# MengLcool/RichSem

Hardware: AMD Instinct MI355X
Metric: training images/sec, RichSem R50 4-scale 1333x800 (MSDeformAttn hot path: 12 fwd + 12 bwd calls per step) (higher is better)
Workload: dtype f32; 1 GPU; configs[1]: R50 4-scale 800x1344 (S=22323), bs=2/GPU, M=8 D=32 L=P=4; per step 6x E(Lq=22323) + 6x Dd(Lq=1092), forward and backward, 12 distinct per-layer tensor sets; loc-init; loc=init, images_per_gpu=2, parallelism=dp1 (replicas, no collective)

## Files before the change

richsem_amd/csrc/msda_rps.h:

```cpp
#pragma once

#include <algorithm>
#include <atomic>
#include <vector>

#include "msda_common.h"

namespace msda {

constexpr int kRpsThreads = 768;
constexpr int kRpsWaves = kRpsThreads / 64;
constexpr int kRpsMaxPx = 256;
constexpr int kRpsPpq = (kRpsMaxPx + kRpsThreads / 4 - 1) / (kRpsThreads / 4);
constexpr int kRpsRpl = 2;
constexpr int kRpsChunk = kRpsRpl * kRpsThreads;
constexpr int kRpsSumStride = 36;
constexpr int kRpsSegShift = 3;
constexpr int kRpsMaxSegs = kRpsMaxPx + (kRpsChunk >> kRpsSegShift);
constexpr int kRpsMaxL = 4;
constexpr int kRpsMaxUnits = 448;
constexpr int kRpsD = 32;
constexpr int kRpsPad = 32;
constexpr int kRpsDummyWgs = 2048, kRpsDummyBytes = kRpsDummyWgs * 1024;
constexpr int kRpsMaxRuns = 320;
constexpr int kRpsRunSearch = 256;
static_assert(kRpsRunSearch < kRpsMaxRuns && 2 * kRpsRunSearch >= kRpsMaxRuns, "run search");
constexpr int kRpsQpBits = 19;
static_assert(kRpsMaxPx <= 256, "record code: the base-grid index has 8 bits (bits 19..26), the tile kernel masks it with 0xFF");

struct RpsLevel {
    int H, W, start;
    int TH, TW, nty, ntx;
    int bin0;
    int nslab;
    int atomic;
    float inv_TH, inv_TW;
};

struct alignas(16) RpsRec {
    unsigned code;
    float lh, lw, a;
};

struct RpsGeom {
    int N, S, M, Lq, L, P;
    int nunits, ppx;
    int bins_per_pair, nbins;
    RpsLevel lv[kRpsMaxL];
    unsigned units[kRpsMaxUnits];
    unsigned *ctr;
    unsigned long long *bin_state;
    uint2 *runs;
    int max_runs;
    int route_threads;
    unsigned entries_cap;
    struct RpsRec *entries;
    int lut_r[kRpsMaxL], lut_c[kRpsMaxL], lut_n;
    int seg_shift;
    float *dummy;
    unsigned long long *stamps;
};

struct alignas(16) RpsEnt {
    float lh;
    float hwa, lwa;
    unsigned row;
};

struct RpsLds {
    int item_slot[2];
    int wave_tot[16];
    int n_segs, pad[3];
    int uhist[16];
    uint2 runs[kRpsMaxRuns];
    unsigned long long stamp_last, stamp_acc[14];
    int offs[kRpsMaxPx + 4];
    unsigned short seg[kRpsMaxSegs + 16];
    RpsEnt ent[kRpsChunk];
    RpsRec meta[kRpsChunk];
    unsigned short slot[kRpsChunk];
    double sum[kRpsMaxPx * kRpsSumStride];
    float vtile[kRpsMaxPx * kRpsD];
};
static_assert(sizeof(RpsLds) <= 160 * 1024, "rps: LDS budget");

__device__ __forceinline__ int rps_wave_scan(int v)
{
    v += __builtin_amdgcn_update_dpp(0, v, 0x111, 0xF, 0xF, true);
    v += __builtin_amdgcn_update_dpp(0, v, 0x112, 0xF, 0xF, true);
    v += __builtin_amdgcn_update_dpp(0, v, 0x114, 0xF, 0xF, true);
    v += __builtin_amdgcn_update_dpp(0, v, 0x118, 0xF, 0xF, true);
    v += __builtin_amdgcn_update_dpp(0, v, 0x142, 0xA, 0xF, false);
    v += __builtin_amdgcn_update_dpp(0, v, 0x143, 0xC, 0xF, false);
    return v;
}

#define RPS_STAMP(i)                                                                   \
    if (kStamps && g.stamps && threadIdx.x == 0) {                                     \
        const unsigned long long now_ = __builtin_amdgcn_s_memtime();                  \
        S->stamp_acc[i] += now_ - S->stamp_last;                                       \
        S->stamp_last = now_;                                                          \
    }

__device__ __forceinline__ unsigned rps_lut_row(const RpsLevel &v, int r)
{
    const int h_low = r - 1, br = max(h_low, 0);
    const int ty = (int)(((float)br + 0.5f) * v.inv_TH);
    const int R0 = ty * v.TH;
    const unsigned gr = (unsigned)(h_low - R0 + 1);
    const unsigned inr = (h_low >= 0 ? 1u : 0u) | (h_low + 1 < v.H ? 2u : 0u);
    return gr | inr << 6 | (unsigned)(ty * v.ntx * v.nslab) << 8;
}
__device__ __forceinline__ unsigned rps_lut_col(const RpsLevel &v, int c)
{
    const int w_low = c - 1, bc = max(w_low, 0);
    const int tx = (int)(((float)bc + 0.5f) * v.inv_TW);
    const int C0 = tx * v.TW, C1 = min(v.W, C0 + v.TW);
    const unsigned gc = (unsigned)(w_low - C0 + 1);
    const unsigned inc = (w_low >= 0 ? 1u : 0u) | (w_low + 1 < v.W ? 2u : 0u);
    const unsigned gw = (unsigned)(C1 - C0 + 1);
    return gc | inc << 6 | (unsigned)(tx * v.nslab) << 8 | gw << 17;
}

constexpr int kRpsRouteThreadsMax = 1024;
static_assert(kRpsMaxUnits <= 512, "route pass: one thread per bin of a pair");

template <int kRpsRouteThreads, int kL = 0, int kP = 0, bool kStamps = false>
__global__ __launch_bounds__(kRpsRouteThreads, 4) void rps_route_kernel(const float *__restrict__ loc, const float *__restrict__ aw,
                                                                     float *__restrict__ grad_value, float *__restrict__ grad_loc,
                                                                     float *__restrict__ grad_aw, const RpsGeom g)
{
    __shared__ unsigned hist[kRpsMaxUnits], base[512];
    __shared__ unsigned wtot[kRpsRouteThreads / kWave];
    __shared__ unsigned sink[kWave];
    extern __shared__ unsigned rps_lut[];
    const int tid = threadIdx.x, lane = tid & (kWave - 1), wave = tid / kWave;
    const int B = g.bins_per_pair;
    const int L = kL ? kL : g.L;
    {
        const int gtid = blockIdx.x * blockDim.x + tid, gsz = gridDim.x * blockDim.x;
        if (gtid < 8) g.ctr[gtid] = 0u;
        if (tid < kWave) sink[tid] = 0u;
        const int row4 = g.M * kRpsD / 4;
        for (int l = 0; l < L; ++l) {
            const RpsLevel &v = g.lv[l];
            for (int i = tid; i <= v.H; i += kRpsRouteThreads) rps_lut[g.lut_r[l] + i] = rps_lut_row(v, i);
            for (int i = tid; i <= v.W; i += kRpsRouteThreads) rps_lut[g.lut_c[l] + i] = rps_lut_col(v, i);
            if (!v.atomic) {
                const int nb = v.nty * v.W + v.ntx * v.H;
                for (int b = 0; b < g.N; ++b) {
                    float4 *dst = reinterpret_cast<float4 *>(grad_value) + (size_t)(b * g.S + v.start) * row4;
                    for (int i = gtid; i < nb * row4; i += gsz) {
                        const int k = i / row4, c = i - k * row4;
                        int px;
                        if (k < v.nty * v.W) {
                            const int ty = k / v.W;
                            px = ty * v.TH * v.W + (k - ty * v.W);
                        } else {
                            const int k2 = k - v.nty * v.W, tx = k2 / v.H;
                            px = (k2 - tx * v.H) * v.W + tx * v.TW;
                        }
                        dst[(size_t)px * row4 + c] = make_float4(0.f, 0.f, 0.f, 0.f);
                    }
                }
                continue;
            }
            const int n4 = v.H * v.W * row4;
            for (int b = 0; b < g.N; ++b) {
                float4 *dst = reinterpret_cast<float4 *>(grad_value) + (size_t)(b * g.S + v.start) * row4;
                for (int i = gtid; i < n4; i += gsz) dst[i] = make_float4(0.f, 0.f, 0.f, 0.f);
            }
        }
    }
    const int P = kP ? kP : g.P, LP = L * P;
    const int qpw = P <= 4 ? 16 : (P <= 8 ? 8 : (P <= 16 ? 4 : (P <= 32 ? 2 : 1)));
    const int ql = lane / P, pp = lane - ql * P;
    const int qpb = qpw * (kRpsRouteThreads / kWave);
    const int qblocks = (g.Lq + qpb - 1) / qpb;
    const int pairs = g.N * g.M;
    const int n_items = pairs * qblocks;
    const unsigned long long lt_mask = (1ull << lane) - 1ull;
    unsigned long long st_acc[8] = {0, 0, 0, 0, 0, 0, 0, 0}, st_last = kStamps && g.stamps ? __builtin_amdgcn_s_memtime() : 0ull;
#define RPS_RSTAMP(i)                                                  \
    if (kStamps && g.stamps) {                                         \
        const unsigned long long now_ = __builtin_amdgcn_s_memtime();  \
        st_acc[i] += now_ - st_last;                                   \
        st_last = now_;                                                \
    }
    float2 xy[kRpsMaxL];
    const int step_pair = (int)(gridDim.x % (unsigned)pairs), step_qb = (int)(gridDim.x / (unsigned)pairs);
    auto item_point = [&](int item_, int pair_, int qb_, bool &live_, int &q_) {
        const int b_ = pair_ / g.M, m_ = pair_ - b_ * g.M;
        q_ = qb_ * qpb + wave * qpw + ql;
        live_ = item_ < n_items && ql < qpw && pp < P && q_ < g.Lq;
        return (unsigned)(((b_ * g.Lq + (live_ ? q_ : 0)) * g.M + m_) * LP + min(pp, P - 1));
    };
    auto request_xy = [&](int item_, int pair_, int qb_) {
        bool live_;
        int q_;
        const unsigned pt0_ = item_point(item_, pair_, qb_, live_, q_);
#pragma unroll
        for (int l = 0; l < kRpsMaxL; ++l) xy[l] = *reinterpret_cast<const float2 *>(loc + 2u * (pt0_ + (unsigned)(min(l, L - 1) * P)));
    };
    int pair = (int)(blockIdx.x % (unsigned)pairs), qb = (int)(blockIdx.x / (unsigned)pairs);
    request_xy(blockIdx.x, pair, qb);
    unsigned long long p_old = 0ull;
    unsigned p_first = 0u, p_cnt = 0u;
    size_t p_gb = 0;
    for (int item = blockIdx.x; item < n_items; item += gridDim.x) {
        for (int i = tid; i < B; i += kRpsRouteThreads) hist[i] = 0u;
        bool live;
        int q;
        const unsigned pt0 = item_point(item, pair, qb, live, q);
        int n_pair = pair + step_pair, n_qb = qb + step_qb;
        if (n_pair >= pairs) {
            n_pair -= pairs;
            ++n_qb;
        }
        n_qb = min(n_qb, qblocks - 1);
        __syncthreads();
        RPS_RSTAMP(1)
        unsigned word[kRpsMaxL];
        unsigned inmap[kRpsMaxL];
        float lh[kRpsMaxL], lw[kRpsMaxL];
        unsigned re[kRpsMaxL], ce[kRpsMaxL];
        unsigned valid_m = 0u, asked_m = 0u, matched_m = 0u;
        unsigned dropped = 0u;
#pragma unroll
        for (int l = 0; l < kRpsMaxL; ++l) {
            lh[l] = lw[l] = 0.f;
            re[l] = ce[l] = 0u;
            if (l >= L) continue;
            const RpsLevel &v = g.lv[l];
            const float Hf = (float)v.H, Wf = (float)v.W;
            const float h_im = xy[l].y * Hf - 0.5f, w_im = xy[l].x * Wf - 0.5f;
            const bool valid = live && h_im > -1.f && w_im > -1.f && h_im < Hf && w_im < Wf;
            valid_m |= valid ? 1u << l : 0u;
            const float hf = floorf(h_im), wf = floorf(w_im);
            lh[l] = h_im - hf;
            lw[l] = w_im - wf;
            dropped |= live && !valid ? 1u << l : 0u;
            re[l] = rps_lut[g.lut_r[l] + (valid ? (int)hf + 1 : 0)];
            ce[l] = rps_lut[g.lut_c[l] + (valid ? (int)wf + 1 : 0)];
        }
        request_xy(item + (int)gridDim.x, n_pair, n_qb);
        float at[kRpsMaxL];
#pragma unroll
        for (int l = 0; l < kRpsMaxL; ++l) at[l] = aw[pt0 + (unsigned)(min(l, L - 1) * P)];
        int ob[kRpsMaxL], lead[kRpsMaxL], lb[kRpsMaxL];
        unsigned own_rank[kRpsMaxL], lt_cnt[kRpsMaxL], n_match[kRpsMaxL];
#pragma unroll
        for (int l = 0; l < kRpsMaxL; ++l) {
            ob[l] = -1;
            lead[l] = 0;
            lb[l] = -1;
            own_rank[l] = lt_cnt[l] = n_match[l] = 0u;
            inmap[l] = 0u;
            word[l] = ~0u;
            if (l >= L) continue;
            const RpsLevel &v = g.lv[l];
            const int ns = v.nslab;
            const int slab = ns > 1 ? uni(qb % ns) : 0;
            ob[l] = (valid_m >> l & 1u) ? v.bin0 + slab + (int)(re[l] >> 8) + (int)((ce[l] >> 8) & 511u) : -1;
            const unsigned inr = (re[l] >> 6) & 3u, inc = (ce[l] >> 6) & 3u;
            inmap[l] = ((inr & 1u) ? inc : 0u) | ((inr & 2u) ? inc << 2 : 0u);
            const unsigned long long vote = __ballot(ob[l] >= 0);
            const int ld = vote ? __ffsll((long long)vote) - 1 : 0;
            lb[l] = __builtin_amdgcn_readlane(ob[l], ld);
            const unsigned long long match = __ballot(ob[l] == lb[l]);
            lead[l] = ld;
            matched_m |= ob[l] == lb[l] && lb[l] >= 0 ? 1u << l : 0u;
            lt_cnt[l] = (unsigned)__popcll(match & lt_mask);
            n_match[l] = (unsigned)__popcll(match);
        }
#pragma unroll
        for (int l = 0; l < kRpsMaxL; ++l) {
            const bool is_lead = lane == lead[l] && lb[l] >= 0, other = ob[l] >= 0 && ob[l] != lb[l];
            const bool asked = is_lead || other;
            asked_m |= asked ? 1u << l : 0u;
            own_rank[l] = atomicAdd(asked ? &hist[is_lead ? lb[l] : ob[l]] : &sink[lane], is_lead ? n_match[l] : (other ? 1u : 0u));
        }
#pragma unroll
        for (int l = 0; l < kRpsMaxL; ++l) {
            if (l >= L) continue;
            const unsigned gr = re[l] & 31u, gc = ce[l] & 31u;
            if (!(asked_m >> l & 1u)) own_rank[l] = lt_cnt[l];
            if (ob[l] >= 0) word[l] = (unsigned)ob[l] | (gr * ((ce[l] >> 17) & 31u) + gc) << 23;
        }
        RPS_RSTAMP(2)
        __syncthreads();
        RPS_RSTAMP(3)
        const unsigned cnt = tid < B ? hist[tid] : 0u;
        const unsigned incl = (unsigned)rps_wave_scan((int)cnt);
        if (lane == kWave - 1) wtot[wave] = incl;
        __syncthreads();
        unsigned before = 0u;
#pragma unroll
        for (int w = 0; w < kRpsRouteThreads / kWave; ++w) before += w < wave ? wtot[w] : 0u;
        const unsigned first = (unsigned)item * (unsigned)(qpb * LP) + before + incl - cnt;
        if (cnt) base[tid] = first;
#pragma unroll
        for (int l = 0; l < kRpsMaxL; ++l) {
            if (l >= L) continue;
            unsigned r = own_rank[l];
            const unsigned rl = (unsigned)__builtin_amdgcn_readlane((int)r, lead[l]);
            if ((matched_m >> l & 1u) && lane != lead[l]) r += rl;
            if (word[l] != ~0u) word[l] |= r << 9;
        }
        __syncthreads();
        RPS_RSTAMP(4)
        const size_t gb = (size_t)pair * B + min(tid, B - 1);
        unsigned long long *const scratch64 = reinterpret_cast<unsigned long long *>(g.dummy + (size_t)(blockIdx.x & (kRpsDummyWgs - 1)) * 256) + lane;
        if (p_cnt) g.runs[p_gb * (size_t)g.max_runs + (size_t)min((unsigned)(p_old >> 32), (unsigned)g.max_runs - 1u)] = make_uint2(p_first, (unsigned)p_old);
        const unsigned long long old = atomicAdd(cnt ? g.bin_state + gb * (kRpsPad / 2) : scratch64, cnt ? (1ull << 32) | (unsigned long long)cnt : 0ull);
        const unsigned qp = (unsigned)((live ? q : 0) * P + pp);
        unsigned slot0[kRpsMaxL];
#pragma unroll
        for (int l = 0; l < kRpsMaxL; ++l) slot0[l] = base[word[l] & 511u];
        asm volatile("" : "+v"(at[0]), "+v"(at[1]), "+v"(at[2]), "+v"(at[3]));
#pragma unroll
        for (int l = 0; l < kRpsMaxL; ++l) {
            const unsigned w = word[l];
            if (w != ~0u) {
                const unsigned slot = min(slot0[l] + ((w >> 9) & 16383u), g.entries_cap - 1u);
                const unsigned code = qp | (w >> 23) << kRpsQpBits | inmap[l] << 27 | 0x80000000u;
                g.entries[slot] = RpsRec{code, lh[l], lw[l], at[l]};
            }
        }
        if (__ballot(dropped != 0u)) {
#pragma unroll
            for (int l = 0; l < kRpsMaxL; ++l)
                if (dropped >> l & 1u) {
                    const unsigned pt = pt0 + (unsigned)(l * P);
                    grad_aw[pt] = 0.f;
                    *reinterpret_cast<float2 *>(grad_loc + 2u * pt) = make_float2(0.f, 0.f);
                }
        }
        RPS_RSTAMP(5)
        p_old = old;
        p_first = first;
        p_cnt = cnt;
        p_gb = gb;
        pair = n_pair;
        qb = n_qb;
        RPS_RSTAMP(6)
        __syncthreads();
        RPS_RSTAMP(7)
    }
    if (p_cnt) g.runs[p_gb * (size_t)g.max_runs + (size_t)min((unsigned)(p_old >> 32), (unsigned)g.max_runs - 1u)] = make_uint2(p_first, (unsigned)p_old);
    if (kStamps && g.stamps && tid == 0)
        for (int i = 0; i < 8; ++i) g.stamps[(size_t)(1024 + blockIdx.x) * 16 + i] = st_acc[i];
#undef RPS_RSTAMP
}

typedef float rps_v2f __attribute__((ext_vector_type(2)));
typedef float rps_v4f __attribute__((ext_vector_type(4)));

__device__ __forceinline__ float rps_quad_rotated_sum(float x0, float x1, float x2, float x3)
{
    const float ra = x0 + dpp_f<kDppXor1>(x1);
    const float rb = x2 + dpp_f<kDppXor1>(x3);
    return ra + dpp_f<kDppXor2>(rb);
}

template <typename TV>
struct RpsRow;
template <>
struct RpsRow<float> {
    float4 a, b;
    __device__ __forceinline__ void load(const float *base, unsigned off)
    {
        a = *reinterpret_cast<const float4 *>(reinterpret_cast<const char *>(base) + off);
        b = *reinterpret_cast<const float4 *>(reinterpret_cast<const char *>(base) + off + 64u);
    }
    __device__ __forceinline__ void unpack(rps_v2f (&gq)[4]) const
    {
        gq[0] = (rps_v2f){a.x, a.y}; gq[1] = (rps_v2f){a.z, a.w};
        gq[2] = (rps_v2f){b.x, b.y}; gq[3] = (rps_v2f){b.z, b.w};
    }
};
template <>
struct RpsRow<bf16_t> {
    uint2 a, b;
    __device__ __forceinline__ void load(const bf16_t *base, unsigned off)
    {
        a = *reinterpret_cast<const uint2 *>(reinterpret_cast<const char *>(base) + off);
        b = *reinterpret_cast<const uint2 *>(reinterpret_cast<const char *>(base) + off + 32u);
    }
    __device__ __forceinline__ void unpack(rps_v2f (&gq)[4]) const
    {
        gq[0] = (rps_v2f){__uint_as_float(a.x << 16), __uint_as_float(a.x & 0xFFFF0000u)};
        gq[1] = (rps_v2f){__uint_as_float(a.y << 16), __uint_as_float(a.y & 0xFFFF0000u)};
        gq[2] = (rps_v2f){__uint_as_float(b.x << 16), __uint_as_float(b.x & 0xFFFF0000u)};
        gq[3] = (rps_v2f){__uint_as_float(b.y << 16), __uint_as_float(b.y & 0xFFFF0000u)};
    }
};

template <bool P4, typename TV = float, bool kStamps = false>
__global__ __launch_bounds__(kRpsThreads, kRpsThreads / 256) void rps_tile_kernel(
    const TV *__restrict__ value, const TV *__restrict__ grad_out, TV *__restrict__ grad_value, float *__restrict__ grad_acc,
    float *__restrict__ grad_loc, float *__restrict__ grad_aw, const RpsGeom g)
{
    extern __shared__ __attribute__((aligned(16))) unsigned char smem[];
    RpsLds *S = reinterpret_cast<RpsLds *>(smem);

    const int tid = threadIdx.x, lane = tid & (kWave - 1), wave = tid / kWave;
    const int j4 = tid & 3, quad = tid >> 2;
    const int c_lo = 4 * j4, c_hi = 16 + 4 * j4;
    const float w_ys = (j4 & 2) ? 1.f : -1.f, w_yc = (j4 & 2) ? 0.f : 1.f;
    const unsigned w_xoff = (j4 & 1) ? 8u : 4u;
    const unsigned lane_row = (unsigned)(c_lo * sizeof(TV));
    const int P = P4 ? 4 : g.P;
    const int LP = g.L * P;
    const int row_elems = g.M * kRpsD;
    const int pairs = g.N * g.M;
    const int xq = blockIdx.x & (kXcds - 1);
    const int n_items = g.nunits * g.ppx;
    float *const dummy_w = g.dummy + (size_t)(blockIdx.x & (kRpsDummyWgs - 1)) * 256;
    if (kStamps && g.stamps && tid == 0) {
        for (int i = 0; i < 14; ++i) S->stamp_acc[i] = 0;
        S->stamp_last = __builtin_amdgcn_s_memtime();
    }
    struct Item {
        bool live;
        int l, b, m, H, W, R0, R1, C0, C1, gw, npx;
    };
    auto item_geom = [&](int id) {
        Item it;
        const unsigned unit = (unsigned)uni((int)g.units[min(id, n_items - 1) / g.ppx]);
        const int pr = xq + kXcds * (min(id, n_items - 1) % g.ppx);
        const int pair = min(pr, pairs - 1);
        it.live = id < n_items && pr < pairs;
        it.l = unit & 3;
        const int ty = (unit >> 2) & 63, tx = (unit >> 8) & 63;
        it.b = pair / g.M;
        it.m = pair - it.b * g.M;
        it.H = g.lv[it.l].H;
        it.W = g.lv[it.l].W;
        it.R0 = ty * g.lv[it.l].TH;
        it.R1 = min(it.H, it.R0 + g.lv[it.l].TH);
        it.C0 = tx * g.lv[it.l].TW;
        it.C1 = min(it.W, it.C0 + g.lv[it.l].TW);
        it.gw = it.C1 - it.C0 + 1;
        it.npx = it.live ? (it.R1 - it.R0 + 1) * it.gw : 0;
        return it;
    };
    auto bin_range_raw = [&](int id, unsigned &bin_, unsigned &okm_, unsigned long long &st_) {
        const int idc = min(id, n_items - 1);
        const unsigned unit = g.units[idc / g.ppx];
        const int pair = xq + kXcds * (idc % g.ppx);
        const bool ok = id < n_items && pair < pairs;
        const int l = unit & 3, ty = (unit >> 2) & 63, tx = (unit >> 8) & 63, slab = (unit >> 14) & 255, nslab = (unit >> 22) & 255;
        const unsigned bin_c = ok ? (unsigned)(pair * g.bins_per_pair + g.lv[l].bin0 + (ty * g.lv[l].ntx + tx) * nslab + slab) : 0u;
        st_ = g.bin_state[(size_t)bin_c * (kRpsPad / 2)];
        okm_ = ok ? 0xFFFFFFFFu : 0u;
        bin_ = bin_c | ~okm_;
    };
    auto bin_counts = [&](unsigned long long st_, unsigned okm_, int &n, int &nr) {
        unsigned lo = (unsigned)st_, hi = (unsigned)(st_ >> 32);
        asm volatile("" : "+v"(lo), "+v"(hi));
        n = (int)(min(lo, 0x7FFFFFFFu) & okm_);
        nr = (int)(min(hi, (unsigned)min(g.max_runs, kRpsMaxRuns)) & okm_);
    };
    auto bin_range = [&](int id, unsigned &bin_, int &n, int &nr) {
        const int idc = min(id, n_items - 1);
        const unsigned unit = g.units[idc / g.ppx];
        const int pair = xq + kXcds * (idc % g.ppx);
        const bool ok = id < n_items && pair < pairs;
        const int l = unit & 3, ty = (unit >> 2) & 63, tx = (unit >> 8) & 63, slab = (unit >> 14) & 255, nslab = (unit >> 22) & 255;
        const unsigned bin_c = ok ? (unsigned)(pair * g.bins_per_pair + g.lv[l].bin0 + (ty * g.lv[l].ntx + tx) * nslab + slab) : 0u;
        const unsigned long long st = g.bin_state[(size_t)bin_c * (kRpsPad / 2)];
        const unsigned okm = ok ? 0xFFFFFFFFu : 0u;
        bin_ = bin_c | ~okm;
        n = (int)(min((unsigned)st, 0x7FFFFFFFu) & okm);
        nr = (int)(min((unsigned)(st >> 32), (unsigned)min(g.max_runs, kRpsMaxRuns)) & okm);
    };
    uint2 run_reg = make_uint2(0u, 0u);
    auto load_runs = [&](unsigned bin_, int nr) {
        const int i = min(tid, max(uni(nr) - 1, 0));
        const unsigned b_ = (unsigned)uni((int)bin_);
        run_reg = g.runs[(size_t)(b_ == 0xFFFFFFFFu ? 0u : b_) * g.max_runs + i];
    };
    auto park_runs = [&]() {
        if (tid < kRpsMaxRuns) S->runs[tid] = run_reg;
    };
    RpsRec n_rec[kRpsRpl];
    auto fetch_recs = [&](int n_, int nr_, int ch) {
        const int n = uni(n_), nr = uni(nr_);
        const int T = max((nr + kWave - 1) / kWave, 1);
        const bool s_ok = lane * T < nr;
        const unsigned sy = S->runs[min(lane * T, max(nr - 1, 0))].y;
        const int k_last = max(n - 1, 0);
#pragma unroll
        for (int u = 0; u < kRpsRpl; ++u) {
            const int kb = ch * kRpsChunk + u * kRpsThreads + wave * kWave;
            const unsigned k = (unsigned)min(kb + lane, k_last);
            const unsigned k_lo = (unsigned)min(kb, k_last), k_hi = (unsigned)min(kb + kWave - 1, k_last);
            const int c_lo = __popcll(__ballot(s_ok && sy <= k_lo)) - 1, c_hi = __popcll(__ballot(s_ok && sy <= k_hi)) - 1;
            const int ra = max(c_lo, 0) * T, rb = min((max(c_hi, 0) + 1) * T, nr);
            int r = ra;
            for (int step = rb - ra > 1 ? 1 << (31 - __builtin_clz(rb - ra - 1)) : 0; step > 0; step >>= 1) {
                const int cand = r + step;
                if (cand < rb && S->runs[cand].y <= k) r = cand;
            }
            const uint2 run = S->runs[r];
            n_rec[u] = g.entries[n > 0 ? min(run.x + (k - run.y), g.entries_cap - 1u) : 0u];
        }
    };
    float4 nv[kRpsPpq][2];
    auto fetch_rows = [&](const Item &it) {
#pragma unroll
        for (int r = 0; r < kRpsPpq; ++r) {
            const int px = min(quad + r * (kRpsThreads / 4), max(it.npx - 1, 0));
            const int gr_ = px / it.gw, gc_ = px - gr_ * it.gw;
            const int prow_ = min(it.R0 + gr_, it.H - 1), pcol_ = min(it.C0 + gc_, it.W - 1);
            const TV *src = value + ((int64_t)(it.b * g.S + g.lv[it.l].start + prow_ * it.W + pcol_) * g.M + it.m) * kRpsD;
            nv[r][0] = ld4(src + c_lo);
            nv[r][1] = ld4(src + c_hi);
        }
    };
    auto store_rows = [&]() {
#pragma unroll
        for (int r = 0; r < kRpsPpq; ++r) {
            const int px = quad + r * (kRpsThreads / 4);
            if (px < kRpsMaxPx) {
                *reinterpret_cast<float4 *>(S->vtile + px * kRpsD + c_lo) = nv[r][0];
                *reinterpret_cast<float4 *>(S->vtile + px * kRpsD + c_hi) = nv[r][1];
            }
        }
    };

    unsigned *const draw_at = tid == 0 ? g.ctr + xq : reinterpret_cast<unsigned *>(dummy_w) + (tid & 255);
    const unsigned draw_by = tid == 0 ? 1u : 0u;
    unsigned draw = atomicAdd(draw_at, draw_by);
    if (tid == 0) S->item_slot[0] = (int)draw;
    draw = atomicAdd(draw_at, draw_by);
    __syncthreads();
    int item_id = uni(S->item_slot[0]);
    unsigned e_bin;
    int n_ent, n_runs;
    bin_range(item_id, e_bin, n_ent, n_runs);
    e_bin = (unsigned)uni((int)e_bin);
    n_ent = uni(n_ent);
    n_runs = uni(n_runs);
    load_runs(e_bin, n_runs);
    park_runs();
    __syncthreads();
    fetch_recs(n_ent, n_runs, 0);
    Item it = item_geom(item_id);
    int par = 0;
    fetch_rows(it);
    for (int i = tid; i < kRpsMaxPx * kRpsSumStride / 2; i += kRpsThreads) reinterpret_cast<double2 *>(S->sum)[i] = make_double2(0.0, 0.0);

    while (item_id < n_items) {
        if (tid == 0) S->item_slot[par ^ 1] = (int)draw;
        const int l = it.l, b = it.b, m = it.m, H = it.H, W = it.W, R0 = it.R0, R1 = it.R1, C0 = it.C0, C1 = it.C1, gw = it.gw;
        const int npx = it.npx;
        const int n_chunks = it.live ? (n_ent + kRpsChunk - 1) / kRpsChunk : 0;
        const int bq0 = b * g.Lq;
        float *const vt = S->vtile;
        __syncthreads();
        const int next_id = uni(S->item_slot[par ^ 1]);
        unsigned next_bin, next_ok;
        unsigned long long next_st;
        int next_n = 0, next_runs = 0;
        bin_range_raw(next_id, next_bin, next_ok, next_st);
        const Item nit = item_geom(next_id);
        store_rows();
        RPS_STAMP(0)

        for (int ch = 0; ch < n_chunks; ++ch) {
            const int n_here = min(kRpsChunk, n_ent - ch * kRpsChunk);
            for (int i = tid; i <= npx; i += kRpsThreads) S->offs[i] = 0;
            int pbase[kRpsRpl], pos[kRpsRpl];
#pragma unroll
            for (int u = 0; u < kRpsRpl; ++u) {
                pos[u] = -1;
                S->meta[u * kRpsThreads + tid] = n_rec[u];
            }
            if (ch == 0) draw = atomicAdd(draw_at, draw_by);
            __syncthreads();
            RPS_STAMP(1)
#pragma unroll
            for (int u = 0; u < kRpsRpl; ++u) {
                pbase[u] = (int)((n_rec[u].code >> kRpsQpBits) & 0xFFu);
                if (u * kRpsThreads + tid < n_here) pos[u] = atomicAdd(&S->offs[pbase[u]], 1);
            }
            __syncthreads();
            RPS_STAMP(2)

            {
                const int sh = g.seg_shift;
                int c = 0, v = 0, incl = 0, n_full = 0, part = 0, pslot = 0, n0 = 0, incl0 = 0, rank = 0, mycnt = 0;
                if (tid < kRpsMaxPx) {
                    c = tid < npx ? S->offs[tid] : 0;
                    v = c | ((c + (1 << sh) - 1) >> sh) << 16;
                    n_full = c >> sh;
                    part = c & ((1 << sh) - 1);
                    pslot = part ? 3 - ((part - 1) >> (sh - 2)) : -1;
                    n0 = n_full + (pslot == 0 ? 1 : 0);
                    incl = rps_wave_scan(v);
                    incl0 = rps_wave_scan(n0);
                    if (lane == kWave - 1) S->wave_tot[wave] = incl;
                    mycnt = __builtin_amdgcn_readlane(incl0, kWave - 1);
                    const unsigned long long lt = (1ull << lane) - 1ull;
#pragma unroll
                    for (int k = 1; k < 4; ++k) {
                        const unsigned long long bk = __ballot(pslot == k);
                        if (pslot == k) rank = __popcll(bk & lt);
                        if (lane == k) mycnt = __popcll(bk);
                    }
                    if (lane < 4) S->uhist[wave * 4 + lane] = mycnt;
                }
                __syncthreads();
                if (tid < kRpsMaxPx) {
                    int base = 0;
#pragma unroll
                    for (int w = 0; w < kRpsMaxPx / kWave; ++w) base += w < wave ? S->wave_tot[w] : 0;
                    const int excl = base + incl - v;
                    if (tid <= npx) S->offs[tid] = excl & 0xFFFF;
                    if (tid == kRpsMaxPx - 1) {
                        if (npx == kRpsMaxPx) S->offs[npx] = (base + incl) & 0xFFFF;
                        S->n_segs = (base + incl) >> 16;
                    }
                    int sbk[4], run_ = 0;
#pragma unroll
                    for (int k = 0; k < 4; ++k) {
                        int tot = 0, mine_before = 0;
#pragma unroll
                        for (int w = 0; w < kRpsMaxPx / kWave; ++w) {
                            const int x = S->uhist[w * 4 + k];
                            tot += x;
                            mine_before += w < wave ? x : 0;
                        }
                        sbk[k] = run_ + mine_before;
                        run_ += tot;
                    }
                    const int at0 = sbk[0] + incl0 - n0;
                    const int atp = (pslot == 1 ? sbk[1] : (pslot == 2 ? sbk[2] : sbk[3])) + rank;
                    for (int sgm = 0; sgm < n_full; ++sgm) S->seg[at0 + sgm] = (unsigned short)(tid | sgm << 8);
                    if (pslot == 0) S->seg[at0 + n_full] = (unsigned short)(tid | n_full << 8);
                    else if (pslot > 0) S->seg[atp] = (unsigned short)(tid | n_full << 8);
                }
            }
            __syncthreads();
            RPS_STAMP(3)

#pragma unroll
            for (int u = 0; u < kRpsRpl; ++u)
                if (pos[u] >= 0) {
                    const int e = pos[u] + S->offs[pbase[u]];
                    const unsigned qp = n_rec[u].code & ((1u << kRpsQpBits) - 1u);
                    const int q = P4 ? (int)(qp >> 2) : (int)(qp / (unsigned)P);
                    const float lwa = n_rec[u].lw * n_rec[u].a;
                    S->ent[e] = RpsEnt{n_rec[u].lh, (1.f - n_rec[u].lw) * n_rec[u].a, lwa, (unsigned)((bq0 + q) * g.M + m) * (unsigned)(kRpsD * sizeof(TV))};
                    S->slot[u * kRpsThreads + tid] = (unsigned short)e;
                }
            __syncthreads();
            RPS_STAMP(4)

            const int n_segs = uni(S->n_segs);
            for (int u0 = wave * 16; u0 < n_segs; u0 += kRpsWaves * 16) {
                unsigned long long wt0 = 0, wt1 = 0, wt2 = 0;
                if (kStamps && g.stamps && tid == 0) wt0 = __builtin_amdgcn_s_memtime();
                const int un = u0 + (lane >> 2);
                if (un < n_segs) {
                    const unsigned sc = S->seg[un];
                    const int my_p = (int)(sc & 0xFFu);
                    int e = S->offs[my_p] + (int)((sc >> 8) << g.seg_shift);
                    const int e1 = min(e + (1 << g.seg_shift), S->offs[my_p + 1]);
                    const int lr = my_p / gw, lc = my_p - lr * gw;
                    const int r0 = max(lr - 1, 0) * gw, c0 = max(lc - 1, 0);
                    rps_v2f v[4][4];
                    {
                        const int row_hi = lr * gw - r0, col_hi = lc - c0;
                        const int row_same = (j4 & 2) ? row_hi : 0, row_flip = row_hi - row_same;
                        const int col_same = (j4 & 1) ? col_hi : 0, col_flip = col_hi - col_same;
                        const float *const v00 = vt + (r0 + c0) * kRpsD;
#pragma unroll
                        for (int r = 0; r < 4; ++r) {
                            const float *const src = v00 + (((r & 2) ? row_flip : row_same) + ((r & 1) ? col_flip : col_same)) * kRpsD;
                            const float4 a0 = *reinterpret_cast<const float4 *>(src + c_lo);
                            const float4 a1 = *reinterpret_cast<const float4 *>(src + c_hi);
                            v[r][0] = (rps_v2f){a0.x, a0.y}; v[r][1] = (rps_v2f){a0.z, a0.w};
                            v[r][2] = (rps_v2f){a1.x, a1.y}; v[r][3] = (rps_v2f){a1.z, a1.w};
                        }
                    }
                    rps_v4f macc[8];
#pragma unroll
                    for (int m_ = 0; m_ < 8; ++m_) macc[m_] = (rps_v4f){0.f, 0.f, 0.f, 0.f};
#define RPS_POINT(ROW, CF, EP)                                                                                                   \
    {                                                                                                                            \
        const float wj = __builtin_fmaf(w_ys, CF.x, w_yc) * CF.y;                                                                \
        rps_v2f gq[4];                                                                                                           \
        ROW.unpack(gq);                                                                                                          \
        _Pragma("unroll") for (int c = 0; c < 4; ++c)                                                                            \
        {                                                                                                                        \
            macc[2 * c] = __builtin_amdgcn_mfma_f32_4x4x1f32(wj, gq[c].x, macc[2 * c], 0, 0, 0);                                 \
            macc[2 * c + 1] = __builtin_amdgcn_mfma_f32_4x4x1f32(wj, gq[c].y, macc[2 * c + 1], 0, 0, 0);                         \
        }                                                                                                                        \
        float d[4];                                                                                                              \
        _Pragma("unroll") for (int k = 0; k < 4; ++k)                                                                            \
        {                                                                                                                        \
            rps_v2f t = gq[0] * v[k][0];                                                                                         \
            t += gq[1] * v[k][1];                                                                                                \
            t += gq[2] * v[k][2];                                                                                                \
            t += gq[3] * v[k][3];                                                                                                \
            d[k] = t.x + t.y;                                                     \
        }                                                                                                                        \
                                               \
        *RPS_LDS(float, (EP) + 4u * (unsigned)j4) = rps_quad_rotated_sum(d[0], d[1], d[2], d[3]);                                \
    }
#define RPS_ROW(OFF, ROW) ROW.load(grad_out, (OFF) + lane_row);
#define RPS_OFF(EP) (*RPS_LDS(const unsigned, (EP) + 12u))
#define RPS_LDS(T, A) (reinterpret_cast<__attribute__((address_space(3))) T *>((size_t)(A)))
                    unsigned ent_lds = (unsigned)(size_t)(__attribute__((address_space(3))) char *)(S->ent);
                    asm volatile("" : "+v"(ent_lds));
                    unsigned ep = ent_lds + (unsigned)e * 16u;
                    const unsigned ep_end = ent_lds + (unsigned)e1 * 16u, ep_last = ep_end - 16u;
                    if (kStamps && g.stamps && wave == 0) {
                        int len = e1 - e;
                        for (int o = 32; o > 0; o >>= 1) len = max(len, __shfl_xor(len, o));
                        if (tid == 0) S->stamp_acc[13] += (unsigned long long)len;
                    }
#define RPS_CF(EP) make_float2(*RPS_LDS(const float, EP), *RPS_LDS(const float, (EP) + w_xoff))
                    unsigned offA = RPS_OFF(ep), offB = RPS_OFF(min(ep + 16u, ep_last));
                    float2 cA = RPS_CF(ep), cB = RPS_CF(min(ep + 16u, ep_last));
                    RpsRow<TV> gA, gB;
                    RPS_ROW(offA, gA)
                    if (kStamps && g.stamps && tid == 0) wt1 = __builtin_amdgcn_s_memtime();
                    for (; ep + 16u < ep_end; ep += 32u) {
                        RPS_ROW(offB, gB)
                        const unsigned nA = min(ep + 32u, ep_last), nB = min(ep + 48u, ep_last);
                        offA = RPS_OFF(nA);
                        const float2 cA2 = RPS_CF(nA);
                        RPS_POINT(gA, cA, ep)
                        RPS_ROW(offA, gA)
                        offB = RPS_OFF(nB);
                        const float2 cB2 = RPS_CF(nB);
                        RPS_POINT(gB, cB, ep + 16u)
                        cA = cA2;
                        cB = cB2;
                    }
                    if (ep < ep_end) RPS_POINT(gA, cA, ep)
#undef RPS_CF
#undef RPS_LDS
#undef RPS_OFF
#undef RPS_ROW
#undef RPS_POINT
                    if (kStamps && g.stamps && tid == 0) wt2 = __builtin_amdgcn_s_memtime();
#pragma unroll
                    for (int k = 0; k < 4; ++k) {
                        const bool ok = (k >= 2 || lr >= 1) && ((k & 1) || lc >= 1);
                        if (ok) {
                            double *dst = S->sum + (my_p - (k < 2 ? gw : 0) - ((k & 1) ? 0 : 1)) * kRpsSumStride + j4;
#pragma unroll
                            for (int m_ = 0; m_ < 8; ++m_) atomicAdd(dst + 4 * m_, (double)macc[m_][k]);
                        }
                    }
                }
                if (kStamps && g.stamps && tid == 0 && wt1) {
                    const unsigned long long wt3 = __builtin_amdgcn_s_memtime();
                    S->stamp_acc[9] += wt1 - wt0;
                    S->stamp_acc[10] += wt2 - wt1;
                    S->stamp_acc[11] += wt3 - wt2;
                    S->stamp_acc[12] += 1;
                }
            }
            const bool last_chunk = ch + 1 == n_chunks;
            bin_counts(next_st, next_ok, next_n, next_runs);
            load_runs(next_bin, next_runs);
            fetch_recs(n_ent, n_runs, min(ch + 1, n_chunks - 1));
            __syncthreads();
            if (last_chunk) park_runs();
            RPS_STAMP(5)

            float ga_[kRpsRpl], gx_[kRpsRpl], gy_[kRpsRpl];
            unsigned pt_[kRpsRpl];
            bool mine_[kRpsRpl];
#pragma unroll
            for (int u = 0; u < kRpsRpl; ++u) {
                const int k = min(u * kRpsThreads + tid, n_here - 1);
                const RpsRec r = S->meta[k];
                float4 d = *reinterpret_cast<const float4 *>(S->ent + S->slot[k]);
                const unsigned in = r.code >> 27;
                if (!(in & 1u)) d.x = 0.f;
                if (!(in & 2u)) d.y = 0.f;
                if (!(in & 4u)) d.z = 0.f;
                if (!(in & 8u)) d.w = 0.f;
                const float lh = r.lh, lw = r.lw, hh = 1.f - lh, hw = 1.f - lw;
                const float s_a = hh * hw * d.x + hh * lw * d.y + lh * hw * d.z + lh * lw * d.w;
                const float s_w = hh * (d.y - d.x) + lh * (d.w - d.z);
                const float s_h = hw * (d.z - d.x) + lw * (d.w - d.y);
                const unsigned qp = r.code & ((1u << kRpsQpBits) - 1u);
                const unsigned q = P4 ? qp >> 2 : qp / (unsigned)P, pp = qp - q * (unsigned)P;
                pt_[u] = (unsigned)((bq0 + (int)q) * g.M + m) * (unsigned)LP + (unsigned)(l * P) + pp;
                mine_[u] = u * kRpsThreads + tid < n_here && (r.code >> 31);
                ga_[u] = s_a;
                gx_[u] = (float)W * s_w * r.a;
                gy_[u] = (float)H * s_h * r.a;
            }
#pragma unroll
            for (int u = 0; u < kRpsRpl; ++u) {
                *(mine_[u] ? grad_aw + pt_[u] : dummy_w + lane) = ga_[u];
                *(mine_[u] ? reinterpret_cast<float2 *>(grad_loc + 2u * pt_[u]) : reinterpret_cast<float2 *>(dummy_w) + lane) = make_float2(gx_[u], gy_[u]);
            }
            RPS_STAMP(6)
        }
        if (n_chunks == 0) {
            draw = atomicAdd(draw_at, draw_by);
            bin_counts(next_st, next_ok, next_n, next_runs);
            load_runs(next_bin, next_runs);
            __syncthreads();
            park_runs();
        }
        fetch_rows(nit);
        __syncthreads();
        fetch_recs(next_n, next_runs, 0);
        if (tid == 0 && e_bin != 0xFFFFFFFFu) g.bin_state[(size_t)e_bin * (kRpsPad / 2)] = 0ull;
        if (!g.lv[l].atomic) {
#pragma unroll
            for (int r = 0; r < kRpsPpq; ++r) {
                const int px = quad + r * (kRpsThreads / 4);
                const int pxc = min(px, kRpsMaxPx - 1);
                const int gr = pxc / gw, gc = pxc - gr * gw;
                const int prow = R0 + gr, pcol = C0 + gc;
                const bool interior = px < npx && gr >= 1 && gc >= 1 && prow < R1 && pcol < C1;
                double *src = S->sum + pxc * kRpsSumStride + j4;
                const int64_t px_off = ((int64_t)(b * g.S + g.lv[l].start + prow * W + pcol) * g.M + m) * kRpsD;
                TV *const dst = interior ? grad_value + px_off : reinterpret_cast<TV *>(dummy_w) + 4 * lane - c_lo;
                st4(dst + c_lo, make_float4((float)src[0], (float)src[4], (float)src[8], (float)src[12]));
                st4(interior ? dst + c_hi : dst + c_lo, make_float4((float)src[16], (float)src[20], (float)src[24], (float)src[28]));
                if (interior) {
#pragma unroll
                    for (int k = 0; k < 8; ++k) src[4 * k] = 0.0;
                }
            }
            const int c32 = tid & 31;
            const int64_t tile_base = ((int64_t)(b * g.S + g.lv[l].start) * g.M + m) * kRpsD + c32;
            const int gh = R1 - R0 + 1, n_border = npx ? 2 * (gw + gh) - 4 : 0;
            for (int k = tid >> 5; k < n_border; k += kRpsThreads / 32) {
                const int k2 = k - 2 * gw;
                const int pr = k < gw ? 0 : (k2 < 0 ? gh - 1 : 1 + (k2 >> 1));
                const int pc = k < gw ? k : (k2 < 0 ? k - gw : ((k2 & 1) ? gw - 1 : 0));
                const int row = R0 + pr, col = C0 + pc;
                double *const sp = S->sum + (pr * gw + pc) * kRpsSumStride + (c32 & 16) + 4 * (c32 & 3) + ((c32 & 15) >> 2);
                const float x = (float)*sp;
                *sp = 0.0;
                if (row < H && col < W && x != 0.f) atomicAdd(grad_acc + tile_base + (int64_t)(row * W + col) * row_elems, x);
            }
        } else if (n_chunks > 0) {
            const int c32 = tid & 31;
            const int64_t tile_base = ((int64_t)(b * g.S + g.lv[l].start) * g.M + m) * kRpsD + c32;
            for (int p = tid >> 5; p < npx; p += kRpsThreads / 32) {
                const int pr = p / gw, row = R0 + pr, col = C0 + (p - pr * gw);
                double *const sp = S->sum + p * kRpsSumStride + (c32 & 16) + 4 * (c32 & 3) + ((c32 & 15) >> 2);
                const float x = (float)*sp;
                *sp = 0.0;
                if (row < H && col < W && x != 0.f) atomicAdd(grad_acc + tile_base + (int64_t)(row * W + col) * row_elems, x);
            }
        }
        __syncthreads();
        RPS_STAMP(7)
        item_id = next_id;
        e_bin = (unsigned)uni((int)next_bin);
        n_ent = uni(next_n);
        n_runs = uni(next_runs);
        it = nit;
        par ^= 1;
    }
    if (kStamps && g.stamps && tid == 0) {
        const unsigned long long now_ = __builtin_amdgcn_s_memtime();
        S->stamp_acc[8] += now_ - S->stamp_last;
        for (int i = 0; i < 14; ++i) g.stamps[(size_t)blockIdx.x * 16 + i] = S->stamp_acc[i];
    }
}

__global__ __launch_bounds__(256) void rps_round_kernel(const float *__restrict__ acc, bf16_t *__restrict__ grad_value, const RpsGeom g)
{
    const int gtid = blockIdx.x * blockDim.x + threadIdx.x, gsz = gridDim.x * blockDim.x;
    const int row4 = g.M * kRpsD / 4;
    for (int l = 0; l < g.L; ++l) {
        const RpsLevel &v = g.lv[l];
        const int nb = v.nty * v.W + v.ntx * v.H;
        const int n4 = (v.atomic ? v.H * v.W : nb) * row4;
        for (int b = 0; b < g.N; ++b) {
            const size_t base = (size_t)(b * g.S + v.start) * row4 * 4;
            for (int i = gtid; i < n4; i += gsz) {
                size_t at = (size_t)i;
                if (!v.atomic) {
                    const int k = i / row4, c = i - k * row4;
                    int px;
                    if (k < v.nty * v.W) {
                        const int ty = k / v.W;
                        px = ty * v.TH * v.W + (k - ty * v.W);
                    } else {
                        const int k2 = k - v.nty * v.W, tx = k2 / v.H;
                        px = (k2 - tx * v.H) * v.W + tx * v.TW;
                    }
                    at = (size_t)px * row4 + c;
                }
                st4(grad_value + base + 4 * at, *reinterpret_cast<const float4 *>(acc + base + 4 * at));
            }
        }
    }
}

struct RpsOptions {
    std::atomic<int> tile{16};
    std::atomic<int> max_chunks{12};
    std::atomic<int> route_wgs{2};
    std::atomic<int> order{0};
    std::atomic<int> seg_shift{4};
};
inline RpsOptions &rps_options()
{
    static RpsOptions o;
    return o;
}

struct RpsPlan {
    bool ok = false;
    RpsGeom g{};
    size_t max_entries = 0;
};

inline RpsPlan plan_rps(int N, int S, int M, int D, int L, int Lq, int P, const int64_t *shapes, const int64_t *lsi)
{
    RpsPlan pl;
    if (D != kRpsD || L < 1 || L > kRpsMaxL || P < 1 || P > 64) return pl;
    int64_t pre = 0;
    bool tiles_s = true;
    for (int l = 0; l < L; ++l) {
        tiles_s = tiles_s && lsi[l] == pre;
        pre += shapes[2 * l] * shapes[2 * l + 1];
        if (shapes[2 * l] >= 32768 || shapes[2 * l + 1] >= 32768) return pl;
    }
    if (!tiles_s || pre != S) return pl;
    const int64_t n_pts = (int64_t)N * Lq * M * L * P;
    if (n_pts >= ((int64_t)1 << 30) || (int64_t)Lq * P >= ((int64_t)1 << kRpsQpBits)) return pl;
    RpsGeom &g = pl.g;
    g.N = N; g.S = S; g.M = M; g.Lq = Lq; g.L = L; g.P = P;
    g.seg_shift = std::max(kRpsSegShift, std::min(11, rps_options().seg_shift.load()));
    g.ppx = (N * M + kXcds - 1) / kXcds;
    const int tmax = std::max(1, rps_options().tile.load() - 1), max_chunks = std::max(1, rps_options().max_chunks.load());
    struct U { unsigned code; int64_t cost; };
    std::vector<U> units;
    int bins = 0;
    for (int l = 0; l < L; ++l) {
        RpsLevel &v = g.lv[l];
        v.H = (int)shapes[2 * l]; v.W = (int)shapes[2 * l + 1]; v.start = (int)lsi[l];
        for (int t = tmax; t >= 1; --t) {
            v.nty = (v.H + t - 1) / t; v.ntx = (v.W + t - 1) / t;
            v.TH = (v.H + v.nty - 1) / v.nty; v.TW = (v.W + v.ntx - 1) / v.ntx;
            v.nty = (v.H + v.TH - 1) / v.TH; v.ntx = (v.W + v.TW - 1) / v.TW;
            if ((v.TH + 1) * (v.TW + 1) <= kRpsMaxPx) break;
        }
        if ((v.TH + 1) * (v.TW + 1) > kRpsMaxPx || v.nty > 64 || v.ntx > 64) return pl;
        const double per_px = (double)Lq * P / ((double)v.H * v.W);
        const int nchunks = (int)(per_px * v.TH * v.TW * 1.05 / kRpsChunk) + 1;
        v.nslab = std::min(255, std::max(1, (nchunks + max_chunks - 1) / max_chunks));
        v.atomic = v.nslab > 1 ? 1 : 0;
        v.inv_TH = 1.0f / (float)v.TH;
        v.inv_TW = 1.0f / (float)v.TW;
        v.bin0 = bins;
        bins += v.nty * v.ntx * v.nslab;
        for (int ty = 0; ty < v.nty; ++ty)
            for (int tx = 0; tx < v.ntx; ++tx)
                for (int sl = 0; sl < v.nslab; ++sl)
                    units.push_back(U{(unsigned)l | (unsigned)ty << 2 | (unsigned)tx << 8 | (unsigned)sl << 14 | (unsigned)v.nslab << 22,
                                      (int64_t)(nchunks + v.nslab - 1) / v.nslab * 16 + 8});
    }
    if (units.size() > (size_t)kRpsMaxUnits) return pl;
    g.lut_n = 0;
    for (int l = 0; l < L; ++l) {
        g.lut_r[l] = g.lut_n;
        g.lut_n += g.lv[l].H + 1;
        g.lut_c[l] = g.lut_n;
        g.lut_n += g.lv[l].W + 1;
    }
    if (rps_options().order.load() == 0) {
        std::stable_sort(units.begin(), units.end(), [](const U &a, const U &b) { return a.cost > b.cost; });
    } else {
        std::vector<int> order;
        for (int l = 0; l < L; ++l)
            if (g.lv[l].nslab == 1) order.push_back(l);
        std::sort(order.begin(), order.end(), [&](int a, int b) { return g.lv[a].nty * g.lv[a].ntx < g.lv[b].nty * g.lv[b].ntx; });
        auto key_of = [&](unsigned code) {
            const int l = code & 3, ty = (code >> 2) & 63, tx = (code >> 8) & 63, nslab = (code >> 22) & 255;
            if (nslab > 1) return (unsigned long long)0;
            const RpsLevel &v = g.lv[l];
            const double cy = (std::min(v.H, ty * v.TH + v.TH) + ty * v.TH) * 0.5 / v.H, cx = (std::min(v.W, tx * v.TW + v.TW) + tx * v.TW) * 0.5 / v.W;
            unsigned long long key = 1ull << 60;
            int shift = 42;
            for (int k : order) {
                const RpsLevel &u = g.lv[k];
                unsigned long long part = 0;
                if (u.nty * u.ntx <= v.nty * v.ntx || k == l) {
                    const int uy = k == l ? ty : std::min(u.nty - 1, (int)(cy * u.H / u.TH)), ux = k == l ? tx : std::min(u.ntx - 1, (int)(cx * u.W / u.TW));
                    part = (unsigned long long)((uy + 1) << 7 | (ux + 1));
                }
                key |= part << shift;
                shift -= 14;
                if (k == l) break;
            }
            return key;
        };
        std::stable_sort(units.begin(), units.end(), [&](const U &a, const U &b) {
            const unsigned long long ka = key_of(a.code), kb = key_of(b.code);
            return ka != kb ? ka < kb : a.cost > b.cost;
        });
    }
    g.nunits = (int)units.size();
    for (int i = 0; i < g.nunits; ++i) g.units[i] = units[i].code;
    g.bins_per_pair = bins;
    g.nbins = bins * N * M;
    const int qpw = P <= 4 ? 16 : (P <= 8 ? 8 : (P <= 16 ? 4 : (P <= 32 ? 2 : 1)));
    g.route_threads = 512;
    g.max_runs = (Lq + qpw * 8 - 1) / (qpw * 8);
    if (g.max_runs > kRpsMaxRuns) {
        g.route_threads = kRpsRouteThreadsMax;
        g.max_runs = (Lq + qpw * 16 - 1) / (qpw * 16);
    }
    if (g.max_runs > kRpsMaxRuns) return pl;
    const int qpb = qpw * (g.route_threads / kWave);
    pl.max_entries = (size_t)N * M * g.max_runs * (size_t)qpb * L * P;
    if (pl.max_entries >= ((size_t)1 << 32)) return pl;
    pl.ok = true;
    return pl;
}

}
```

Measured before the change: 730.0 img/s.

## Enlarge RPS tiles, add cost-based tile search, reload records instead of LDS meta

Raises the per-tile pixel cap from 256 to 312 and widens the base-grid index field in the record code to 9 bits, dropping the validity bit. The scan, segment encoding and histogram are widened to match. A host-side search now enumerates tile grid shapes and picks the one with the lowest estimated chunk and slab cost. The per-chunk LDS meta array is removed: record indices are kept in registers and the records are re-read from global memory just before accumulation. This frees LDS and shared-memory traffic at the cost of an extra global load, and larger tiles change the work balance across units.

```diff
diff --git a/richsem_amd/csrc/msda_rps.h b/richsem_amd/csrc/msda_rps.h
--- a/richsem_amd/csrc/msda_rps.h
+++ b/richsem_amd/csrc/msda_rps.h
@@ -10,7 +10,9 @@
 
 constexpr int kRpsThreads = 768;
 constexpr int kRpsWaves = kRpsThreads / 64;
-constexpr int kRpsMaxPx = 256;
+constexpr int kRpsMaxPx = 312;
+constexpr int kRpsMaxSide = 31;
+constexpr int kRpsScanThreads = (kRpsMaxPx + 63) / 64 * 64, kRpsScanWaves = kRpsScanThreads / 64;
 constexpr int kRpsPpq = (kRpsMaxPx + kRpsThreads / 4 - 1) / (kRpsThreads / 4);
 constexpr int kRpsRpl = 2;
 constexpr int kRpsChunk = kRpsRpl * kRpsThreads;
@@ -26,7 +28,10 @@
 constexpr int kRpsRunSearch = 256;
 static_assert(kRpsRunSearch < kRpsMaxRuns && 2 * kRpsRunSearch >= kRpsMaxRuns, "run search");
 constexpr int kRpsQpBits = 19;
-static_assert(kRpsMaxPx <= 256, "record code: the base-grid index has 8 bits (bits 19..26), the tile kernel masks it with 0xFF");
+constexpr int kRpsPxBits = 9;
+static_assert(kRpsMaxPx <= 1 << kRpsPxBits && kRpsQpBits + kRpsPxBits + 4 == 32, "record code: qp | base-grid index | corners");
+static_assert(kRpsMaxPx <= kRpsMaxSide * kRpsMaxSide && kRpsScanThreads <= kRpsThreads && kRpsScanWaves * 4 <= 32, "tile grid");
+static_assert(kRpsChunk < 1 << 16, "a list's length and a chunk's unit count share a 32-bit word in the scan; slot[] is 16 bits wide");
 
 struct RpsLevel {
     int H, W, start;
@@ -71,16 +76,15 @@
     int item_slot[2];
     int wave_tot[16];
     int n_segs, pad[3];
-    int uhist[16];
+    int uhist[32];
     uint2 runs[kRpsMaxRuns];
     unsigned long long stamp_last, stamp_acc[14];
-    int offs[kRpsMaxPx + 4];
-    unsigned short seg[kRpsMaxSegs + 16];
+    int offs[kRpsScanThreads + 4];
+    unsigned seg[kRpsMaxSegs + 16];
     RpsEnt ent[kRpsChunk];
-    RpsRec meta[kRpsChunk];
     unsigned short slot[kRpsChunk];
-    double sum[kRpsMaxPx * kRpsSumStride];
-    float vtile[kRpsMaxPx * kRpsD];
+    alignas(16) double sum[kRpsMaxPx * kRpsSumStride];
+    alignas(16) float vtile[kRpsMaxPx * kRpsD];
 };
 static_assert(sizeof(RpsLds) <= 160 * 1024, "rps: LDS budget");
 
@@ -323,7 +327,7 @@
             const unsigned w = word[l];
             if (w != ~0u) {
                 const unsigned slot = min(slot0[l] + ((w >> 9) & 16383u), g.entries_cap - 1u);
-                const unsigned code = qp | (w >> 23) << kRpsQpBits | inmap[l] << 27 | 0x80000000u;
+                const unsigned code = qp | (w >> 23) << kRpsQpBits | inmap[l] << (kRpsQpBits + kRpsPxBits);
                 g.entries[slot] = RpsRec{code, lh[l], lw[l], at[l]};
             }
         }
@@ -485,6 +489,7 @@
         if (tid < kRpsMaxRuns) S->runs[tid] = run_reg;
     };
     RpsRec n_rec[kRpsRpl];
+    unsigned n_idx[kRpsRpl];
     auto fetch_recs = [&](int n_, int nr_, int ch) {
         const int n = uni(n_), nr = uni(nr_);
         const int T = max((nr + kWave - 1) / kWave, 1);
@@ -504,7 +509,8 @@
                 if (cand < rb && S->runs[cand].y <= k) r = cand;
             }
             const uint2 run = S->runs[r];
-            n_rec[u] = g.entries[n > 0 ? min(run.x + (k - run.y), g.entries_cap - 1u) : 0u];
+            n_idx[u] = n > 0 ? min(run.x + (k - run.y), g.entries_cap - 1u) : 0u;
+            n_rec[u] = g.entries[n_idx[u]];
         }
     };
     float4 nv[kRpsPpq][2];
@@ -574,16 +580,13 @@
             for (int i = tid; i <= npx; i += kRpsThreads) S->offs[i] = 0;
             int pbase[kRpsRpl], pos[kRpsRpl];
 #pragma unroll
-            for (int u = 0; u < kRpsRpl; ++u) {
-                pos[u] = -1;
-                S->meta[u * kRpsThreads + tid] = n_rec[u];
-            }
+            for (int u = 0; u < kRpsRpl; ++u) pos[u] = -1;
             if (ch == 0) draw = atomicAdd(draw_at, draw_by);
             __syncthreads();
             RPS_STAMP(1)
 #pragma unroll
             for (int u = 0; u < kRpsRpl; ++u) {
-                pbase[u] = (int)((n_rec[u].code >> kRpsQpBits) & 0xFFu);
+                pbase[u] = min((int)((n_rec[u].code >> kRpsQpBits) & ((1u << kRpsPxBits) - 1u)), kRpsMaxPx - 1);
                 if (u * kRpsThreads + tid < n_here) pos[u] = atomicAdd(&S->offs[pbase[u]], 1);
             }
             __syncthreads();
@@ -592,7 +595,7 @@
             {
                 const int sh = g.seg_shift;
                 int c = 0, v = 0, incl = 0, n_full = 0, part = 0, pslot = 0, n0 = 0, incl0 = 0, rank = 0, mycnt = 0;
-                if (tid < kRpsMaxPx) {
+                if (tid < kRpsScanThreads) {
                     c = tid < npx ? S->offs[tid] : 0;
                     v = c | ((c + (1 << sh) - 1) >> sh) << 16;
                     n_full = c >> sh;
@@ -613,14 +616,14 @@
                     if (lane < 4) S->uhist[wave * 4 + lane] = mycnt;
                 }
                 __syncthreads();
-                if (tid < kRpsMaxPx) {
+                if (tid < kRpsScanThreads) {
                     int base = 0;
 #pragma unroll
-                    for (int w = 0; w < kRpsMaxPx / kWave; ++w) base += w < wave ? S->wave_tot[w] : 0;
+                    for (int w = 0; w < kRpsScanWaves; ++w) base += w < wave ? S->wave_tot[w] : 0;
                     const int excl = base + incl - v;
                     if (tid <= npx) S->offs[tid] = excl & 0xFFFF;
-                    if (tid == kRpsMaxPx - 1) {
-                        if (npx == kRpsMaxPx) S->offs[npx] = (base + incl) & 0xFFFF;
+                    if (tid == kRpsScanThreads - 1) {
+                        if (npx == kRpsScanThreads) S->offs[npx] = (base + incl) & 0xFFFF;
                         S->n_segs = (base + incl) >> 16;
                     }
                     int sbk[4], run_ = 0;
@@ -628,7 +631,7 @@
                     for (int k = 0; k < 4; ++k) {
                         int tot = 0, mine_before = 0;
 #pragma unroll
-                        for (int w = 0; w < kRpsMaxPx / kWave; ++w) {
+                        for (int w = 0; w < kRpsScanWaves; ++w) {
                             const int x = S->uhist[w * 4 + k];
                             tot += x;
                             mine_before += w < wave ? x : 0;
@@ -638,9 +641,9 @@
                     }
                     const int at0 = sbk[0] + incl0 - n0;
                     const int atp = (pslot == 1 ? sbk[1] : (pslot == 2 ? sbk[2] : sbk[3])) + rank;
-                    for (int sgm = 0; sgm < n_full; ++sgm) S->seg[at0 + sgm] = (unsigned short)(tid | sgm << 8);
-                    if (pslot == 0) S->seg[at0 + n_full] = (unsigned short)(tid | n_full << 8);
-                    else if (pslot > 0) S->seg[atp] = (unsigned short)(tid | n_full << 8);
+                    for (int sgm = 0; sgm < n_full; ++sgm) S->seg[at0 + sgm] = (unsigned)(tid | sgm << 16);
+                    if (pslot == 0) S->seg[at0 + n_full] = (unsigned)(tid | n_full << 16);
+                    else if (pslot > 0) S->seg[atp] = (unsigned)(tid | n_full << 16);
                 }
             }
             __syncthreads();
@@ -666,8 +669,8 @@
                 const int un = u0 + (lane >> 2);
                 if (un < n_segs) {
                     const unsigned sc = S->seg[un];
-                    const int my_p = (int)(sc & 0xFFu);
-                    int e = S->offs[my_p] + (int)((sc >> 8) << g.seg_shift);
+                    const int my_p = (int)(sc & 0xFFFFu);
+                    int e = S->offs[my_p] + (int)((sc >> 16) << g.seg_shift);
                     const int e1 = min(e + (1 << g.seg_shift), S->offs[my_p + 1]);
                     const int lr = my_p / gw, lc = my_p - lr * gw;
                     const int r0 = max(lr - 1, 0) * gw, c0 = max(lc - 1, 0);
@@ -767,6 +770,13 @@
                     S->stamp_acc[12] += 1;
                 }
             }
+            RpsRec c_rec[kRpsRpl];
+#pragma unroll
+            for (int u = 0; u < kRpsRpl; ++u) {
+                unsigned ix = n_idx[u];
+                asm volatile("" : "+v"(ix));
+                c_rec[u] = g.entries[ix];
+            }
             const bool last_chunk = ch + 1 == n_chunks;
             bin_counts(next_st, next_ok, next_n, next_runs);
             load_runs(next_bin, next_runs);
@@ -781,9 +791,9 @@
 #pragma unroll
             for (int u = 0; u < kRpsRpl; ++u) {
                 const int k = min(u * kRpsThreads + tid, n_here - 1);
-                const RpsRec r = S->meta[k];
+                const RpsRec r = c_rec[u];
                 float4 d = *reinterpret_cast<const float4 *>(S->ent + S->slot[k]);
-                const unsigned in = r.code >> 27;
+                const unsigned in = r.code >> (kRpsQpBits + kRpsPxBits);
                 if (!(in & 1u)) d.x = 0.f;
                 if (!(in & 2u)) d.y = 0.f;
                 if (!(in & 4u)) d.z = 0.f;
@@ -795,7 +805,7 @@
                 const unsigned qp = r.code & ((1u << kRpsQpBits) - 1u);
                 const unsigned q = P4 ? qp >> 2 : qp / (unsigned)P, pp = qp - q * (unsigned)P;
                 pt_[u] = (unsigned)((bq0 + (int)q) * g.M + m) * (unsigned)LP + (unsigned)(l * P) + pp;
-                mine_[u] = u * kRpsThreads + tid < n_here && (r.code >> 31);
+                mine_[u] = u * kRpsThreads + tid < n_here;
                 ga_[u] = s_a;
                 gx_[u] = (float)W * s_w * r.a;
                 gy_[u] = (float)H * s_h * r.a;
@@ -943,23 +953,38 @@
     g.N = N; g.S = S; g.M = M; g.Lq = Lq; g.L = L; g.P = P;
     g.seg_shift = std::max(kRpsSegShift, std::min(11, rps_options().seg_shift.load()));
     g.ppx = (N * M + kXcds - 1) / kXcds;
-    const int tmax = std::max(1, rps_options().tile.load() - 1), max_chunks = std::max(1, rps_options().max_chunks.load());
+    const int tile_opt = rps_options().tile.load();
+    const int tmax = tile_opt >= 16 ? kRpsMaxSide - 1 : std::max(1, tile_opt - 1), max_chunks = std::max(1, rps_options().max_chunks.load());
     struct U { unsigned code; int64_t cost; };
     std::vector<U> units;
     int bins = 0;
     for (int l = 0; l < L; ++l) {
         RpsLevel &v = g.lv[l];
         v.H = (int)shapes[2 * l]; v.W = (int)shapes[2 * l + 1]; v.start = (int)lsi[l];
-        for (int t = tmax; t >= 1; --t) {
-            v.nty = (v.H + t - 1) / t; v.ntx = (v.W + t - 1) / t;
-            v.TH = (v.H + v.nty - 1) / v.nty; v.TW = (v.W + v.ntx - 1) / v.ntx;
-            v.nty = (v.H + v.TH - 1) / v.TH; v.ntx = (v.W + v.TW - 1) / v.TW;
-            if ((v.TH + 1) * (v.TW + 1) <= kRpsMaxPx) break;
-        }
-        if ((v.TH + 1) * (v.TW + 1) > kRpsMaxPx || v.nty > 64 || v.ntx > 64) return pl;
         const double per_px = (double)Lq * P / ((double)v.H * v.W);
-        const int nchunks = (int)(per_px * v.TH * v.TW * 1.05 / kRpsChunk) + 1;
-        v.nslab = std::min(255, std::max(1, (nchunks + max_chunks - 1) / max_chunks));
+        auto chunks_of = [&](int th, int tw) { return (int)(per_px * th * tw * 1.05 / kRpsChunk) + 1; };
+        auto slabs_of = [&](int nchunks) { return std::min(255, std::max(1, (nchunks + max_chunks - 1) / max_chunks)); };
+        int64_t best = -1;
+        v.TH = v.TW = v.nty = v.ntx = 0;
+        for (int nty = 1; nty <= std::min(64, v.H); ++nty) {
+            const int th = (v.H + nty - 1) / nty;
+            if (th > tmax || (v.H + th - 1) / th != nty) continue;
+            int tried = 0;
+            for (int ntx = 1; ntx <= std::min(64, v.W) && tried < 4; ++ntx) {
+                const int tw = (v.W + ntx - 1) / ntx;
+                if (tw > tmax || (th + 1) * (tw + 1) > kRpsMaxPx || (v.W + tw - 1) / tw != ntx) continue;
+                ++tried;
+                const int nch = chunks_of(th, tw);
+                const int64_t cost = (int64_t)nty * ntx * (5 * slabs_of(nch) + 2 * nch);
+                if (best < 0 || cost < best) {
+                    best = cost;
+                    v.TH = th; v.TW = tw; v.nty = nty; v.ntx = ntx;
+                }
+            }
+        }
+        if (best < 0) return pl;
+        const int nchunks = chunks_of(v.TH, v.TW);
+        v.nslab = slabs_of(nchunks);
         v.atomic = v.nslab > 1 ? 1 : 0;
         v.inv_TH = 1.0f / (float)v.TH;
         v.inv_TW = 1.0f / (float)v.TW;
@@ -979,6 +1004,7 @@
         g.lut_c[l] = g.lut_n;
         g.lut_n += g.lv[l].W + 1;
     }
+    if (g.lut_n > kRpsMaxL * 2 * 962) return pl;
     if (rps_options().order.load() == 0) {
         std::stable_sort(units.begin(), units.end(), [](const U &a, const U &b) { return a.cost > b.cost; });
     } else {
```

Result: faster. 740.3 img/s (median of 6 runs) (+1.4%).
